# RandomMike1280/AlphaZero-Reversi

Hardware: AMD Instinct MI355X
Metric: self-play board-steps/sec @ 800 sims/move, 8x8 Reversi (higher is better)
Workload: dtype u64 rules + f32 NN (fp32 as 2-part f16 split on MFMA)

## Files before the change

### alphazero-reversi_amd/csrc/rvz_engine_host.h

```cpp
#pragma once
#include <hip/hip_runtime.h>
#include <stdint.h>

#include <string>
#include <utility>
#include <vector>

#include "../../include/rvz.h"
#include "rvz_host.hip.h"
#include "rvz_search.hip.h"

using namespace rvz;

struct rvz_engine {
    rvz_config cfg;
    int BS, NSQ, NPOL, E, M;
    hipStream_t stream = nullptr;
    int next_batch = 0;
    int32_t* live_buf = nullptr;
    unsigned long long* live_total = nullptr;
    int live_dirty = 0;
    int searching = 0;
    int pending = 0;
    const float* pend_policy = nullptr;
    const float* pend_value = nullptr;
    int pend_is_logits = 0;
    int64_t counters[2] = {0, 0};
    View v;
    unsigned long long* stats_buf = nullptr;
    int timing = 0;
    std::vector<hipEvent_t> ev_pool;
    size_t ev_used = 0;
    std::vector<std::pair<int, size_t>> ev_marks;
    std::vector<void*> allocs;
    std::string err;
    unsigned long long* tab = nullptr;
    unsigned* tclaim = nullptr;
    unsigned* tgen = nullptr;
    int64_t tslots = 0;
    int tmaxd = 0;
    const void* tab_blob = nullptr;
    double gate_frac = -1.0, gate_us = 0.0, gate_late_us = 0.0;
    int32_t* noise_err = nullptr;
    void* open_buf = nullptr;
};

#define RVZ_HIP(call, e)                                                                   \
    do {                                                                                   \
        hipError_t _s = (call);                                                            \
        if (_s != hipSuccess) {                                                            \
            (e)->err = std::string(#call) + ": " + hipGetErrorString(_s);                  \
            return RVZ_EHIP;                                                               \
        }                                                                                  \
    } while (0)

static int launch_check(rvz_engine* e, const char* what) {
    hipError_t s = hipGetLastError();
    if (s != hipSuccess) {
        e->err = std::string(what) + ": " + hipGetErrorString(s);
        return RVZ_EHIP;
    }
    e->counters[1] += 1;
    return RVZ_OK;
}

static int grid_games(int G) { return (G + WPB - 1) / WPB; }

template <class... P, class... A>
static void launch_games_unchecked(rvz_engine* e, void (*k8)(P...), void (*k6)(P...), A... args) {
    launch_bs_unchecked(e->BS, k8, k6, dim3(grid_games(e->v.G)), dim3(WPB * WAVE), e->stream,
                        args...);
}
template <class... P, class... A>
static int launch_games(rvz_engine* e, const char* what, void (*k8)(P...), void (*k6)(P...),
                        A... args) {
// ... 27 lines not shown
```

### alphazero-reversi_amd/csrc/rvz_play.hip

```cpp
#include <hip/hip_runtime.h>
#include <math.h>
#include <stdint.h>
#include <stdio.h>
#include <stdlib.h>

#include <string>
#include <vector>

#include "../../include/rvz.h"
#include "rvz_engine_host.h"
#include "rvz_h2.hip.h"
#include "rvz_host.hip.h"
#include "rvz_play.hip.h"
#include "rvz_search.hip.h"
#include "rvz_trace.h"

using namespace rvz;


__global__ void k_table_bump(unsigned* gen) {
    if (threadIdx.x == 0) atomicAdd(gen, 1u);
}

int table_bump(rvz_engine* e) {
    if (!e->tgen) return RVZ_OK;
    hipLaunchKernelGGL(k_table_bump, dim3(1), dim3(64), 0, e->stream, e->tgen);
    RVZ_HIP(hipGetLastError(), e);
    return RVZ_OK;
}

void table_free(rvz_engine* e) {
    for (void* p : {(void*)e->tab, (void*)e->tclaim, (void*)e->tgen})
        if (p) (void)hipFree(p);
    e->tab = nullptr;
    e->tclaim = nullptr;
    e->tgen = nullptr;
    e->tslots = 0;
    e->tab_blob = nullptr;
}

extern "C" {

int rvz_play_gate(rvz_engine* e, double fraction, double timeout_us, double late_us) {
    if (!e || !(fraction <= 1.0) || !(timeout_us >= 0.0) || !(late_us >= 0.0) ||
        timeout_us > 1e6 || late_us > 1e6) {
        if (e) e->err = "rvz_play_gate: fraction <= 1 (< 0: the default), 0 <= us <= 1e6";
        return RVZ_EINVAL;
    }
    e->gate_frac = fraction;
    e->gate_us = timeout_us;
    e->gate_late_us = late_us;
    return RVZ_OK;
}

int rvz_play_table(rvz_engine* e, int64_t slots, int32_t max_discs) {
    if (!e) return RVZ_EINVAL;
    if (slots != 0 && (slots < 1024 || (slots & (slots - 1)) != 0 || slots > (1ll << 30) ||
                       max_discs < 4)) {
        e->err = "rvz_play_table: slots a power of two in [1024, 2^30] (or 0), max_discs >= 4";
        return RVZ_EINVAL;
    }
    RVZ_HIP(hipStreamSynchronize(e->stream), e);
    if (slots == e->tslots && slots != 0) {
        e->tmaxd = max_discs;
        return table_bump(e);
    }
    table_free(e);
    if (slots == 0) return RVZ_OK;
    const size_t stride = e->BS == 8 ? TabGeo<8>::STRIDE : TabGeo<6>::STRIDE;
    if (hipMalloc(reinterpret_cast<void**>(&e->tab), (size_t)slots * stride * 8) != hipSuccess ||
        hipMalloc(reinterpret_cast<void**>(&e->tclaim), (size_t)slots * 4) != hipSuccess ||
        hipMalloc(reinterpret_cast<void**>(&e->tgen), 4) != hipSuccess) {
        table_free(e);
        e->err = "hipMalloc failed (rvz_play_table)";
        return RVZ_ENOMEM;
    }
    hipError_t st = hipMemset(e->tab, 0, (size_t)slots * stride * 8);
    if (st == hipSuccess) st = hipMemset(e->tclaim, 0, (size_t)slots * 4);
    if (st == hipSuccess) st = hipMemsetD32(e->tgen, 1u, 1);
    if (st == hipSuccess) st = hipDeviceSynchronize();
    if (st != hipSuccess) {
        table_free(e);
        e->err = std::string("rvz_play_table init: ") + hipGetErrorString(st);
        return RVZ_EHIP;
    }
    e->tslots = slots;
    e->tmaxd = max_discs;
    return RVZ_OK;
}

#ifdef RVZ_WALK_STATS
int rvz_play_walk_read(int32_t n_games, uint64_t* out) {
    const int n = n_games < WALK_STATS_MAX ? n_games : WALK_STATS_MAX;
    std::vector<unsigned long long> a, b;
    if (take_rows(g_wtime, n, a) != RVZ_OK || take_rows(g_ftime, n, b) != RVZ_OK) return RVZ_EHIP;
    for (int i = 0; i < n; ++i) {
        for (int k = 0; k < 5; ++k) out[(size_t)i * 9 + k] = a[(size_t)i * 5 + k];
        for (int k = 0; k < 4; ++k) out[(size_t)i * 9 + 5 + k] = b[(size_t)i * 4 + k];
    }
    return RVZ_OK;
}
#endif

struct PlayScratch {
    int64_t q_next, q_done, gate, queue, x, need, work, logits, value, total;
};
static PlayScratch play_scratch(int64_t G, int NSQ, int NPOL) {
    const auto al4 = [](int64_t n) { return (n + 3) / 4 * 4; };
    int64_t at = 0;
    const auto take = [&](int64_t words) { const int64_t o = at; at += al4(words); return o; };
    PlayScratch s;
    s.q_next = take(4);
    s.q_done = take(2 * al4(G));
    s.gate = take(8 * 32);
    s.queue = at;
    s.x = take(G * 3 * NSQ);
    s.need = take(G);
    s.work = take(G * 192);
    s.logits = take(G * NPOL);
    s.value = take(G);
    s.total = at;
    return s;
}
int64_t rvz_play_scratch_size(const rvz_engine* e) {
    if (!e) return RVZ_EINVAL;
    return play_scratch(e->v.G, e->NSQ, e->NPOL).total;
}

#ifndef RVZ_PLAY_GROUP
#define RVZ_PLAY_GROUP 4
#endif
#ifndef RVZ_PLAY_GATE_FRAC
#define RVZ_PLAY_GATE_FRAC 0.8
#endif
#ifndef RVZ_PLAY_GATE_US
#define RVZ_PLAY_GATE_US 400.0
#endif
#ifndef RVZ_PLAY_GATE_LATE_US
#define RVZ_PLAY_GATE_LATE_US 200.0
#endif
extern "C++" {
template <class T>
static int play_launch(rvz_engine* e, const View& v, const PlayArgs& pa) {
    constexpr int F = T::F, BS = T::BS;
    int cus = 0;
    if (hipDeviceGetAttribute(&cus, hipDeviceAttributeMultiprocessorCount, e->cfg.device) !=
            hipSuccess || cus <= 0)
        cus = 256;
    PlayArgs a = pa;
    const int slots = cus * T::OCC;
    dim3 grid;
    if (a.q_next) {
        if (a.gpw <= 0) a.gpw = RVZ_PLAY_GROUP;
        if (a.gpw > play_gpw_max<F, BS>()) a.gpw = play_gpw_max<F, BS>();
        a.n_groups = (v.G + a.gpw - 1) / a.gpw;
        grid = dim3(a.n_groups < slots ? a.n_groups : slots);
        RVZ_HIP(fill32_async(a.q_next, 0u, (size_t)play_scratch(v.G, e->NSQ, e->NPOL).queue,
                             e->stream), e);
    } else {
        if (a.gpw <= 0) a.gpw = (v.G + slots - 1) / slots;
        if (a.gpw > play_gpw_max<F, BS>()) a.gpw = play_gpw_max<F, BS>();
        a.n_groups = (v.G + a.gpw - 1) / a.gpw;
        grid = dim3(a.n_groups);
    }
    PlayCtx ctx;
    ctx.v = v;
    ctx.a = a;
    hipLaunchKernelGGL((k_play<T::F, T::NB, T::CTW, T::PTW, T::BS, T::OCC>), grid, dim3(256), 0,
                       e->stream, ctx);
    return launch_check(e, "k_play");
}
}

#ifdef RVZ_PLAY_TIMING
int rvz_play_timing_read(uint64_t* host, int n) {
    if (hipMemcpyFromSymbol(host, HIP_SYMBOL(g_play_t), (size_t)n * PLAY_T_SLOTS * 8) != hipSuccess)
        return RVZ_EHIP;
    if (hipMemcpyFromSymbol(host + (size_t)n * PLAY_T_SLOTS, HIP_SYMBOL(g_pass_t),
                            (size_t)n * 6 * 8) != hipSuccess)
        return RVZ_EHIP;
    std::vector<unsigned long long> z((size_t)16384 * PLAY_T_SLOTS, 0ull);
    if (hipMemcpyToSymbol(HIP_SYMBOL(g_pass_t), z.data(), (size_t)16384 * 6 * 8) != hipSuccess)
// ... 67 lines not shown
    pa.need = reinterpret_cast<int32_t*>(a->scratch + sc.need);
    pa.work = a->scratch + sc.work;
    pa.logits = a->scratch + sc.logits;
    pa.value = a->scratch + sc.value;
    pa.n_groups = 0;
    pa.gpw = queue ? -a->games_per_workgroup : a->games_per_workgroup;
    const PlayGate gate = play_gate_setting(e, queue);
    pa.gate_frac = gate.frac;
    pa.gate_t = gate.t;
    pa.gate_late = gate.late;
    pa.spin_limit = 1u << 26;
    if (const char* sl = getenv("RVZ_PLAY_SPIN_LIMIT")) pa.spin_limit = (unsigned)strtoul(sl, nullptr, 10);
    pa.single_pass = 1;
    if (const char* sp = getenv("RVZ_PLAY_SINGLE_PASS")) pa.single_pass = atoi(sp) != 0;
    pa.S = e->cfg.num_simulations;
    pa.B = e->cfg.batch_size;
    pa.skip_last = a->skip_last_eval && pa.S > pa.B ? 1 : 0;
    pa.skip_forced = a->skip_forced_roots && pa.skip_last ? 1 : 0;
    pa.plies = a->plies;
    pa.budget = a->ply_budget;
    pa.temperature = a->temperature;
    pa.reset = a->reset ? 1 : 0;
    pa.seeds = a->seeds;
    pa.stride = a->seed_stride;
    pa.ply_ctr = a->plies_done;
    pa.done = a->games_done;
    pa.out_idx = a->out_idx;
    pa.out_p = a->out_p;
    pa.hist = a->hist;
    pa.rows = reinterpret_cast<unsigned long long*>(a->rows_evaluated);
    pa.unread = reinterpret_cast<unsigned long long*>(a->rows_unread);
    pa.roots_unread = reinterpret_cast<unsigned long long*>(a->roots_unread);
    pa.tstats = reinterpret_cast<unsigned long long*>(a->table_stats);
    pa.rec_black = a->rec_black;
    pa.rec_white = a->rec_white;
    pa.rec_side = a->rec_side;
    pa.rec_p = a->rec_p;
    pa.tab = nullptr;
    pa.tclaim = nullptr;
    pa.tgen = nullptr;
    pa.tmask = 0;
    pa.tmaxd = 0;
    if (e->tab) {
        if (e->tab_blob != a->blob) {
            if (e->tab_blob) {
                hipStreamCaptureStatus cs = hipStreamCaptureStatusNone;
                if (hipStreamIsCapturing(e->stream, &cs) == hipSuccess &&
                    cs != hipStreamCaptureStatusNone) {
                    e->err = "rvz_play: another weight blob than the table's while the stream is "
                             "capturing (play once eagerly with this evaluator before capturing)";
                    return RVZ_EINVAL;
                }
                const int r = table_bump(e);
                if (r != RVZ_OK) return r;
            }
            e->tab_blob = a->blob;
        }
        pa.tab = e->tab;
        pa.tclaim = e->tclaim;
        pa.tgen = e->tgen;
        pa.tmask = (unsigned)(e->tslots - 1);
        pa.tmaxd = e->tmaxd;
    }
    e->searching = 0;
    int r = RVZ_EINVAL;
    h2_tile(e->BS, a->filters, [&](auto t) { r = play_launch<decltype(t)>(e, v, pa); });
// ... 5 lines not shown
```

### alphazero-reversi_amd/csrc/rvz_play.hip.h

```cpp
#pragma once
#include <hip/hip_runtime.h>
#include <stdint.h>

#include "rvz_h2.hip.h"
#include "rvz_resnet_common.hip.h"
#include "rvz_search.hip.h"

namespace rvz {
namespace {

struct PlayArgs {
    const float* prm;
    Layout L;
    const uint16_t* blob;
    int n_blocks;
    float* x;
    int32_t* need;
    float* work;
    float* logits;
    float* value;
    float* ovf;
    int gpw, plies, skip_last, reset, S, B;
    double temperature;
    int64_t* seeds;
    int64_t stride;
    int64_t* ply_ctr;
    int64_t* done;
    int32_t* out_idx;
    double* out_p;
    int32_t* hist;
    unsigned long long* rows;
    const int32_t* budget;
    unsigned spin_limit;
    int single_pass;
    unsigned long long* tab;
    unsigned* tclaim;
    const unsigned* tgen;
    unsigned tmask;
    int tmaxd;
    unsigned long long* tstats;
    unsigned long long* unread;
    uint64_t* rec_black;
    uint64_t* rec_white;
    int32_t* rec_side;
    double* rec_p;
    unsigned* q_next;
    unsigned long long* q_done;
    int n_groups;
    unsigned long long* gate;
    unsigned gate_frac;
    unsigned gate_t;
    unsigned gate_late;
    int skip_forced;
    unsigned long long* roots_unread;
};
constexpr int PLAY_GPW_MAX = 64;
template <int F, int BS>
__host__ __device__ constexpr bool play_heads_lds() { return F == 64 && BS == 8; }
template <int F, int BS>
__host__ __device__ constexpr int play_gpw_max() {
    return play_heads_lds<F, BS>() ? 8 : PLAY_GPW_MAX;
}
enum : int { PF_QUEUED = 1, PF_READY = 2, PF_DONE = 4, PF_EVAL = 8, PF_HELD = 16 };
constexpr int32_t ERR_SCHED = 16;

template <int BS>
struct TabGeo {
    static constexpr int NSQ = Geo<BS>::NSQ;
    static constexpr int NG = NSQ + 8;
    static constexpr int STRIDE = (NG + 7) / 8 * 8;
};
constexpr int TAB_PROBES = 8;

__device__ __forceinline__ uint64_t tab_mix(uint64_t z) {
    z ^= z >> 30;
    z *= 0xbf58476d1ce4e5b9ull;
    z ^= z >> 27;
    z *= 0x94d049bb133111ebull;
    return z ^ (z >> 31);
}
__device__ __forceinline__ uint64_t tab_hash(uint64_t P, uint64_t O, uint64_t V) {
    return tab_mix(P ^ tab_mix(O ^ tab_mix(V + 0x9e3779b97f4a7c15ull)));
}
template <int NSQ>
__device__ __forceinline__ uint32_t tab_key_word(int idx, uint64_t P, uint64_t O, uint64_t V) {
    const int k = idx - (NSQ + 2);
    const uint64_t w = k < 2 ? P : (k < 4 ? O : V);
    return (k & 1) ? (uint32_t)(w >> 32) : (uint32_t)w;
}

template <int BS>
__device__ __forceinline__ int tab_read(const unsigned long long* __restrict__ tab, uint32_t sl,
                                         uint32_t gen, uint64_t P, uint64_t O, uint64_t V,
                                         int lane, uint64_t& x0, uint64_t& x1) {
    using T = TabGeo<BS>;
    constexpr int NSQ = T::NSQ, NG = T::NG;
// ... 111 lines not shown
                           __HIP_MEMORY_SCOPE_AGENT);
}
__device__ __forceinline__ void play_gate(unsigned long long* gate, unsigned frac, unsigned t,
                                          unsigned late) {
    unsigned long long* w = gate_line(gate);
    if (late) {
        const unsigned long long t_open =
            __hip_atomic_load(w + 1, __ATOMIC_RELAXED, __HIP_MEMORY_SCOPE_AGENT);
        if (t_open && __builtin_amdgcn_s_memrealtime() - t_open < late) return;
    }
    const unsigned long long running =
        __hip_atomic_load(w + 2, __ATOMIC_RELAXED, __HIP_MEMORY_SCOPE_AGENT);
    if (running < 4) return;
    const unsigned k = max(1u, (unsigned)((running * frac) >> 16));
    const unsigned long long old =
        __hip_atomic_fetch_add(w, 1ull, __ATOMIC_RELAXED, __HIP_MEMORY_SCOPE_AGENT);
    const unsigned r = (unsigned)(old >> 32);
    if ((unsigned)old + 1u >= k) {
        gate_open(w, r);
        return;
    }
    const unsigned long long t0 = __builtin_amdgcn_s_memrealtime();
    for (;;) {
        __builtin_amdgcn_s_sleep(2);
        const unsigned long long v = __hip_atomic_load(w, __ATOMIC_RELAXED, __HIP_MEMORY_SCOPE_AGENT);
        if ((unsigned)(v >> 32) != r) return;
        if (__builtin_amdgcn_s_memrealtime() - t0 > t) {
            gate_open(w, r);
            return;
        }
    }
}

struct PlayCtx {
    View v;
    PlayArgs a;
};
__device__ __forceinline__ int opaque_tid() {
    int t = threadIdx.x;
    asm volatile("" : "+v"(t));
    return t;
}
__device__ __forceinline__ const PlayCtx& play_ctx() {
    const __attribute__((address_space(4))) char* p =
        (const __attribute__((address_space(4))) char*)__builtin_amdgcn_kernarg_segment_ptr();
    asm volatile("" : "+s"(p));
    return *(const PlayCtx*)p;
}

#ifdef RVZ_PLAY_TIMING
constexpr int PLAY_T_SLOTS = 14;
__device__ unsigned long long g_play_t[16384][PLAY_T_SLOTS];
#define PT_NOW(t) const unsigned long long t = __builtin_amdgcn_s_memtime()
#define PT_ADD(i, v) if (tid == 0 && blockIdx.x < 16384) g_play_t[blockIdx.x][i] += (v)
#else
#define PT_NOW(t)
#define PT_ADD(i, v)
#endif

template <int F, int NBOARD, int CTW, int PTW, int BS, int OCC>
__global__ __launch_bounds__(256) __attribute__((amdgpu_waves_per_eu(OCC, OCC)))
void k_play(PlayCtx ctx0) {
    (void)ctx0;
    using WT = WaveTilesH<F, CTW, PTW>;
    constexpr bool ILV = RVZ_H2_ILV && NBOARD == 2 && BS == 8 && PTW == 4 && WT::CG == 2;
    using GH = GeoH<NBOARD, BS, 64 * CTW * H2_TM / F, ILV>;
    using C = CfgH<F, GH::NPIX>;
    constexpr int NPOL = Geo<BS>::NPOL;
    constexpr bool HLDS = play_heads_lds<F, BS>();
    constexpr int GMAX = play_gpw_max<F, BS>();
    constexpr bool PLAY_SINGLE = F == 64 && NBOARD == 2 && BS == 8 && (PTW & 1) == 0 && HLDS;
    constexpr int HROW = heads_in_floats(BS) / 16;
    constexpr int SP_BYTES = WPB * (NPOL + 7) * 8;
    static_assert(heads_in_floats(BS) * 4 <= C::RMAX, "heads rows fit");
    static_assert(SP_BYTES + WPB * 624 * 4 <= C::RMAX, "act / reset scratch fits");
    __shared__ __attribute__((aligned(16))) char smem[C::BYTES];
    __shared__ int st_k[GMAX];
    __shared__ int st_f[GMAX];
    __shared__ int st_p[GMAX];
    __shared__ uint64_t st_bits[GMAX * 3];
    __shared__ uint64_t q_bits[(GMAX + NBOARD) * 3];
    __shared__ __attribute__((aligned(16))) float hin[HLDS ? GMAX * HROW : 4];
    __shared__ int q_rows[GMAX + 16];
    __shared__ int s_nq;
    __shared__ float vpart[4][16];
    __shared__ int s_task[2];
    __shared__ unsigned s_tgen;
    const int tid = threadIdx.x;
    const int wave = __builtin_amdgcn_readfirstlane(tid >> 6);
    int E, G, gpw, queue, task_plies;
    {
        const PlayCtx& c = play_ctx();
        E = c.v.E;
        G = c.v.G;
        gpw = c.a.gpw;
        queue = c.a.q_next != nullptr;
        task_plies = queue ? 1 : c.a.plies;
    }
    bool ovf = false;
    __shared__ unsigned s_cnt[5];
    if (tid < 5) s_cnt[tid] = 0u;
    if (tid == 0) {
        const PlayArgs& a = play_ctx().a;
        s_tgen = a.tab ? __hip_atomic_load(a.tgen, __ATOMIC_RELAXED, __HIP_MEMORY_SCOPE_AGENT) : 0u;
    }
    double* sp = reinterpret_cast<double*>(smem) + wave * (NPOL + 7);
    uint32_t* key = reinterpret_cast<uint32_t*>(smem + SP_BYTES) + wave * 624;
    if constexpr (F >= 128 && BS == 8) {
        const PlayArgs& a = play_ctx().a;
        if (tid == 0 && a.gate_frac > 0) gate_running(a.gate, 1);
    }
    PT_NOW(t_start);
    for (int task_i = 0;; ++task_i) {
        int gi, ply0;
        if (!queue) {
            if (task_i > 0) break;
            gi = blockIdx.x;
            ply0 = 0;
        } else {
            PT_NOW(t_q0);
            if (wave == 0) {
                const PlayCtx& c = play_ctx();
                const PlayArgs& a = c.a;
                const int n = a.n_groups;
                const unsigned plies = (unsigned)a.plies;
                const int rot = (int)((unsigned long long)blockIdx.x * (unsigned)n / gridDim.x);
                int tg = -1, tp = 0;
                bool stop = __hip_atomic_load(c.v.err, __ATOMIC_RELAXED,
                                              __HIP_MEMORY_SCOPE_AGENT) & ERR_SCHED;
                unsigned spins = 0;
                while (!stop) {
                    unsigned long long best = ~0ull;
                    bool left = false;
                    for (int i = tid; i < n; i += 64) {
// ... 96 lines not shown
                            root_meta = v.meta[(size_t)g * v.M];
                            root_n = v.nodes[(size_t)g * v.M].n;
                        } else if (v.memo) {
                            carry = v.carry[g];
                        }
                        if (f & PF_READY) {
                            WT_NOW(ft_e);
                            const ExpIn x = expand_load<BS>(v, g, lane, a.logits, a.value);
                            const int rn =
                                expand_backup_phase<BS>(v, g, lane, x, 1, &root_meta, ab);
                            if (rn >= 0) root_n = rn;
                            f &= ~PF_READY;
                            FT_ADD(0, ft_e);
                        }
                        const int bsz = min(a.B, a.S - k * a.B);
                        const bool unread = a.skip_last && !first && m_nchild(root_meta) >= E - 1;
                        const Forced fz{first && a.skip_forced ? E : 0, a.S, a.B};
                        const int copies = select_phase<BS, float>(v, g, lane, first, bsz, k, root,
                                                                   root_meta, root_n, carry, a.x,
                                                                   a.need, ab, st_bits + 3 * j,
                                                                   unread, fz);
                        if (copies <= -2) {
                            k = E;
                            const int left = -2 - copies;
                            if (lane == 0) {
                                if (left & 255) atomicAdd(&s_cnt[3], (unsigned)(left & 255));
                                if (left >> 8) atomicAdd(&s_cnt[4], 1u);
                            }
                            continue;
                        }
                        ++k;
                        if (copies < 0 && k < E && lane == 0) atomicAdd(&s_cnt[3], 1u);
                        if (copies > 0 && !(k == E && a.skip_last)) {
                            if (a.tab) {
                                const uint64_t P = st_bits[3 * j], O = st_bits[3 * j + 1],
                                               Vb = st_bits[3 * j + 2];
                                WT_NOW(ft_t);
                                const bool hit = __popcll(P | O) <= a.tmaxd &&
                                                 tab_lookup<BS>(a, s_tgen, P, O, Vb, lane, g);
                                WT_ADD(0, ft_t);
                                if (hit) {
                                    __builtin_amdgcn_fence(__ATOMIC_SEQ_CST, "workgroup");
                                    f |= PF_READY;
                                    if (lane == 0) atomicAdd(&s_cnt[1], 1u);
                                    continue;
                                }
                            }
                            f |= PF_QUEUED;
                            break;
                        }
                        continue;
                    }
                    WT_NOW(ft_a);
                    bool over = false;
                    double* outp = a.out_p;
                    if (a.rec_black) {
                        const size_t ri = (size_t)(ply0 + np) * v.G + g;
                        if (lane == 0) {
                            a.rec_black[ri] = v.black[g];
                            a.rec_white[ri] = v.white[g];
                            a.rec_side[ri] = v.status[(size_t)g * 4];
                        }
                        outp = a.rec_p + (size_t)(ply0 + np) * v.G * Geo<BS>::NPOL;
                    }
                    const int idx = act_game<BS>(v, g, lane, sp, (f & PF_READY) ? 1 : 2,
                                                 a.logits, 1, a.value, a.temperature, nullptr, 1,
                                                 a.out_idx, outp, &over);
                    f &= ~PF_READY;
                    int64_t sd = 0;
                    if (lane == 0) {
                        if (idx >= 0) a.ply_ctr[g] += 1;
                        if (a.hist) a.hist[(size_t)(ply0 + np) * v.G + g] = idx;
                        if (a.reset && over) {
                            a.done[g] += 1;
                            sd = a.seeds[g] + a.stride;
                            a.seeds[g] = sd;
                        }
                    }
                    if (a.reset && over) {
                        sd = __shfl(sd, 0);
                        reset_game<BS>(v, g, lane, (uint32_t)(sd & 0xFFFFFFFFll), key);
                    }
                    FT_ADD(1, ft_a);
                    ++np;
                    k = 0;
                    if (np >= task_plies || (a.budget && ply0 + np >= a.budget[g])) {
                        f |= PF_DONE;
                        break;
                    }
                }
                FT_ADD(2, ft_step);
                if (lane == 0) {
                    st_k[j] = k;
                    st_f[j] = f;
                    st_p[j] = np;
                }
            }
            __syncthreads();
            PT_NOW(t_c1);
            PT_ADD(0, t_c1 - t_c0);
            PT_ADD(4, 1);
            if (tid == 0) {
                int n = 0;
                for (int j = 0; j < ng; ++j)
                    if (st_f[j] & PF_QUEUED) ++n;
                int hold = n > NBOARD ? n % NBOARD : 0;
                for (int j = ng - 1; j >= 0; --j) {
                    const int fj = st_f[j];
                    if (!(fj & PF_QUEUED)) continue;
                    if (hold > 0 && !(fj & PF_HELD)) {
                        st_f[j] = fj | PF_HELD;
                        --hold;
                    } else {
                        st_f[j] = (fj & ~PF_HELD) | PF_EVAL;
                    }
                }
                n = 0;
                for (int j = 0; j < ng; ++j)
                    if (st_f[j] & PF_EVAL) {
                        for (int ch = 0; ch < 3; ++ch) q_bits[3 * n + ch] = st_bits[3 * j + ch];
                        q_rows[n++] = g0 + j;
                    }
                for (int i = n; i < n + 16; ++i) q_rows[i] = -1;
                for (int i = 3 * n; i < 3 * (n + NBOARD); ++i) q_bits[i] = 0;
                s_nq = n;
            }
            __syncthreads();
            const int nq = __builtin_amdgcn_readfirstlane(s_nq);
            if (nq == 0) break;
            if (tid == 0) s_cnt[0] += (unsigned)nq;
            PT_NOW(t_c2);

            for (int p0 = 0; p0 < nq; p0 += NBOARD) {
                if constexpr (F >= 128 && BS == 8) {
                    if (play_ctx().a.gate_frac > 0) {
                        if (tid == 0) {
                            const PlayArgs& a = play_ctx().a;
                            play_gate(a.gate, a.gate_frac, a.gate_t, a.gate_late);
                        }
                        __syncthreads();
                    }
                }
                const PlayArgs& a = play_ctx().a;
                PT_NOW(t_p0);
                bool single = false;
                if constexpr (PLAY_SINGLE)
                    single = a.single_pass &&
                             __builtin_amdgcn_readfirstlane(q_rows[p0 + 1]) < 0;
                if (single) {
                    if constexpr (PLAY_SINGLE) {
                        const int t = opaque_tid();
                        ovf |= h2_pass_single<F, CTW, PTW / 2, BS>(
                                   smem, q_bits + 3 * p0, a.prm, a.blob, a.n_blocks, hin, p0, nq,
                                   t, t & 63, __builtin_amdgcn_readfirstlane(t >> 6)) != 0;
                    }
                } else {
                    int gb[NBOARD];
// ... 85 lines not shown
    if (queue && tid == 0) {
        const PlayCtx& c = play_ctx();
        const PlayArgs& a = c.a;
        unsigned spins = 0;
        bool stop = __hip_atomic_load(c.v.err, __ATOMIC_RELAXED, __HIP_MEMORY_SCOPE_AGENT) &
                    ERR_SCHED;
        while (!stop && (int)__hip_atomic_load(a.q_next, __ATOMIC_RELAXED,
                                               __HIP_MEMORY_SCOPE_AGENT) < a.n_groups) {
            __builtin_amdgcn_s_sleep(4);
            ++spins;
            if (spins > a.spin_limit ||
                ((spins & 1023u) == 0 &&
                 (__hip_atomic_load(c.v.err, __ATOMIC_RELAXED, __HIP_MEMORY_SCOPE_AGENT) &
                  ERR_SCHED))) {
                atomicOr(c.v.err, ERR_SCHED);
                stop = true;
            }
        }
    }
    float* ovw = play_ctx().a.ovf;
    if (ovf && ovw) *ovw = 1.0f;
    unsigned long long* rows = play_ctx().a.rows;
    __syncthreads();
    if (rows && tid == 0) atomicAdd(rows, (unsigned long long)s_cnt[0]);
    unsigned long long* ts = play_ctx().a.tstats;
    if (ts && tid == 0) {
        if (s_cnt[1]) atomicAdd(ts, (unsigned long long)s_cnt[1]);
        if (s_cnt[2]) atomicAdd(ts + 1, (unsigned long long)s_cnt[2]);
    }
    unsigned long long* un = play_ctx().a.unread;
    if (un && tid == 0 && s_cnt[3]) atomicAdd(un, (unsigned long long)s_cnt[3]);
    unsigned long long* ur = play_ctx().a.roots_unread;
    if (ur && tid == 0 && s_cnt[4]) atomicAdd(ur, (unsigned long long)s_cnt[4]);
}

}
}
```

### alphazero-reversi_amd/csrc/rvz_search.hip.h

```cpp
#pragma once
#include <hip/hip_runtime.h>
#include <math.h>
#include <stdint.h>

#include "../../include/rvz.h"
#include "rvz_dirichlet.hip.h"
#include "rvz_openings.hip.h"
#include "rvz_philox.hip.h"
#include "rvz_pow.hip.h"
#include "rvz_rules.hip.h"
#include "rvz_wave_dpp.hip.h"

namespace rvz {
namespace {

constexpr int WAVE = 64;
constexpr int WPB = 4;
constexpr int PATH_CAP = 64;
constexpr int RNG_DRAWS = 64;

}

struct Node {
    int32_t n;
// ... 557 lines not shown
            if (leaf_bits) {
                if (lane == 0) {
                    leaf_bits[0] = mine(sim);
                    leaf_bits[1] = theirs(sim);
                    leaf_bits[2] = V;
                }
            } else if (lane < NSQ) {
                XT* row = leaf_x + (size_t)r * 3 * NSQ;
                const uint64_t P = mine(sim), O = theirs(sim);
                row[lane] = (XT)(float)((P >> lane) & 1ull);
                row[NSQ + lane] = (XT)(float)((O >> lane) & 1ull);
                row[2 * NSQ + lane] = (XT)(float)((V >> lane) & 1ull);
            }
            if (lane < plen) v.path[g * PATH_CAP + lane] = path_reg;
            if (lane == 0) {
                v.leaf_legal[g] = V;
                v.leaf_meta[g] = m;
            }
            WT_ADD(4, tl0);
            ab += 3ull * NSQ * sizeof(XT) + 4ull * plen + 12;
            break;
        }
    }
    if (lane == 0) {
        need[g] = copies;
        v.pend[g] = copies;
        v.plen[g] = plen;
    }
    ab += 12;
    return copies;
}

template <int BS>
__device__ __forceinline__ int root_visits(const View& v, int g, int lane) {
    constexpr int NSQ = Geo<BS>::NSQ;
    const Node* nodes = v.nodes + (size_t)g * v.M;
    const uint32_t m0 = v.meta[(size_t)g * v.M];
    const uint64_t V = v.root_legal[g];
    const int nch = m_nchild(m0);
    if (nch == 0 || lane >= NSQ) return 0;
    if (!((V >> lane) & 1ull)) return 0;
    const int idx = __popcll(V & ((1ull << lane) - 1ull));
    return nodes[1 + m_block(m0) * NSQ + idx].n;
}

__device__ __forceinline__ double np_power(double x, double e) {
    if (e == 1.0) return x;
    if (e == 2.0) return x * x;
    if (e == 0.5) return sqrt(x);
    if (e == -1.0) return 1.0 / x;
    if (e == 0.0) return 1.0;
    return rvz_pow::pow_cr(x, e);
}

template <int BS, class Draw>
__device__ __forceinline__ int select_action(int n, int npass, int lane, double* s,
                                             double temperature, Draw&& draw, double& p,
                                             double& ppass, int& drew) {
    constexpr int NSQ = Geo<BS>::NSQ, NPOL = Geo<BS>::NPOL;
    constexpr int NMAIN = NPOL - NPOL % 8;
    const int total = wave_sum_i(lane < NSQ ? n : 0) + npass;
    p = (lane < NSQ && total > 0) ? (double)n / (double)total : 0.0;
    ppass = npass != 0 ? (double)npass / (double)total : 0.0;
    if (temperature > 0.0 && (__any(p != 0.0) || ppass != 0.0)) {
        const double ex = 1.0 / temperature;
        const double t = lane < NSQ ? np_power(p, ex) : 0.0;
// ... 165 lines not shown
```

### alphazero-reversi_amd/rvz/_lib.py

```python
from __future__ import annotations

import ctypes as C
import math
import numbers
import os

import torch

_HERE = os.path.dirname(os.path.abspath(__file__))
LIB_PATH = os.environ.get("RVZ_LIB", os.path.join(_HERE, "librvz.so"))

RVZ_OK, RVZ_DONE = 0, 1
RVZ_LEAF_F32, RVZ_LEAF_BF16 = 0, 1
RVZ_DRAWS = 64
RVZ_SOLVE_MAX_EMPTIES = 14
RVZ_SOLVE_NOT_A_MOVE, RVZ_SOLVE_ABANDONED = -128, -127
RVZ_AB_MAX_DEPTH = 12
RVZ_AB_WIN = 20000
RVZ_AB_HEUR_MAX = 16000


class RvzError(RuntimeError):
    pass

# ... 78 lines not shown
                                            C.c_uint64, C.c_uint64, _P, _P, _P, _P, _P, _P, _P]),
    "rvz_replay_is_weight_scratch_size": (C.c_int64, [C.c_int32]),
    "rvz_replay_is_weight": (C.c_int, [C.c_int32, _P, _P, C.c_double, _P, _P, _P, _P]),
    "rvz_replay_priority_scratch_size": (C.c_int64, [C.c_int32]),
    "rvz_replay_priority": (C.c_int, [C.c_int32, _P, C.c_int32, _P, _P, C.c_double, C.c_double,
                                      C.c_int32, C.c_double, C.c_double, C.c_double, _P, _P, _P,
                                      _P, _P]),
    "rvz_replay_stale_scratch_size": (C.c_int64, [C.c_int32, C.c_int32]),
    "rvz_replay_stale": (C.c_int, [C.c_int32, _P, C.c_int32, C.c_int32, C.c_int32, C.c_int32,
                                   C.c_int32, _P, C.c_int64, _P, _P, _P]),
    "rvz_replay_roots": (C.c_int, [C.c_int32, C.c_int32, _P, _P, C.c_int32, _P, _P, _P, _P, _P,
                                   _P]),
    "rvz_replay_refresh_scratch_size": (C.c_int64, [C.c_int32]),
    "rvz_replay_refresh": (C.c_int, [C.c_int32, C.c_int32, _P, _P, C.c_int32, _P, _P, _P,
                                     C.c_int32, _P, C.c_int64, _P, _P]),
    "rvz_records_scratch_size": (C.c_int64, [C.c_int32, C.c_int32]),
    "rvz_records_games": (C.c_int, [C.c_int32, C.c_int32, C.c_int32, _P, _P, _P, _P, _P, C.c_int32,
                                    _P, _P, _P, _P, _P, _P, _P, _P, _P, _P]),
    "rvz_records_final": (C.c_int, [C.c_int32, C.c_int32, C.c_int32, _P, _P, _P, _P, C.c_int32,
                                    _P, _P, _P, _P, _P, _P, _P]),
    "rvz_openings_scratch_size": (C.c_int64, [C.c_int32, C.c_int32]),
    "rvz_openings": (C.c_int, [C.c_int32, C.c_int32, C.c_int32, _P, _P, _P, _P, _P, _P, _P]),
    "rvz_env_openings": (C.c_int, [_P, C.c_int32, _P, _P, _P, C.c_uint32]),
    "rvz_opening_index": (C.c_int, [C.c_int32, C.c_int32, _P, C.c_uint32, _P, _P]),
    "rvz_loss_scratch_size": (C.c_int64, [C.c_int32, C.c_int32]),
    "rvz_policy_value_loss": (C.c_int, [C.c_int32, C.c_int32, _P, _P, _P, _P, _P, C.c_double,
                                        C.c_double, _P, _P, _P, _P, _P, _P]),
    "rvz_ownership_loss_scratch_size": (C.c_int64, [C.c_int32, C.c_int32]),
    "rvz_ownership_loss": (C.c_int, [C.c_int32, C.c_int32, _P, _P, _P, _P, _P, _P, _P, _P]),
    "rvz_play_scratch_size": (C.c_int64, [_P]),
    "rvz_play": (C.c_int, [_P, _P]),
    "rvz_play_table": (C.c_int, [_P, C.c_int64, C.c_int32]),
    "rvz_play_gate": (C.c_int, [_P, C.c_double, C.c_double, C.c_double]),
    "rvz_counters": (C.c_int, [_P, C.POINTER(C.c_int64)]),
    "rvz_stats_enable": (C.c_int, [_P, C.c_int32]),
    "rvz_stats_read": (C.c_int, [_P, C.POINTER(C.c_int64)]),
    "rvz_timing_enable": (C.c_int, [_P, C.c_int32]),
    "rvz_timing_read": (C.c_int, [_P, C.POINTER(C.c_double), C.POINTER(C.c_int32)]),
    "rvz_tree_nodes": (C.c_int, [_P]),
    "rvz_tree_export": (C.c_int, [_P, _P, _P]),
    "rvz_footprint": (C.c_int, [_P, C.POINTER(C.c_int64), C.POINTER(C.c_int64)]),
    "rvz_resnet_params_size": (C.c_int64, [C.c_int32, C.c_int32, C.c_int32]),
    "rvz_resnet_work_size": (C.c_int64, [C.c_int32]),
    "rvz_resnet_heads_fc": (C.c_int, [C.c_int32, _P, C.c_int32, _P, C.c_int32, C.c_int32, _P, _P,
                                      _P]),
    "rvz_resnet_h2_size": (C.c_int64, [C.c_int32, C.c_int32]),
    "rvz_resnet_h2_weights": (C.c_int, [_P, C.c_int32, C.c_int32, _P, _P]),
    "rvz_resnet_trunk_h2": (C.c_int, [C.c_int32, _P, C.c_int32, _P, _P, C.c_int32, C.c_int32,
                                      _P, _P]),
    "rvz_resnet_fwd_h2": (C.c_int, [C.c_int32, _P, C.c_int32, _P, _P, C.c_int32, C.c_int32, _P,
                                    _P, _P, _P]),
}

_lib = None


class PlayArgs(C.Structure):
    _fields_ = [("params", C.c_void_p), ("blob", C.c_void_p), ("filters", C.c_int32),
                ("blocks", C.c_int32), ("scratch", C.c_void_p), ("ovf", C.c_void_p),
                ("plies", C.c_int32), ("skip_last_eval", C.c_int32), ("reset", C.c_int32),
                ("games_per_workgroup", C.c_int32), ("temperature", C.c_double),
                ("seeds", C.c_void_p), ("seed_stride", C.c_int64), ("plies_done", C.c_void_p),
                ("games_done", C.c_void_p), ("out_idx", C.c_void_p), ("out_p", C.c_void_p),
                ("hist", C.c_void_p), ("rows_evaluated", C.c_void_p),
                ("ply_budget", C.c_void_p), ("table_stats", C.c_void_p),
                ("rec_black", C.c_void_p), ("rec_white", C.c_void_p), ("rec_side", C.c_void_p),
# ... 123 lines not shown
```

### alphazero-reversi_amd/rvz/engine.py

```python
from __future__ import annotations

import ctypes as C
from typing import Callable, Optional, Sequence, Tuple

import torch

from . import _lib
from ._lib import (RVZ_DONE, RVZ_LEAF_BF16, RVZ_LEAF_F32, RvzError, check, check_board_size,
                   ptr)

U64 = 0xFFFFFFFFFFFFFFFF
SOLVE_MAX_EMPTIES = _lib.RVZ_SOLVE_MAX_EMPTIES
SOLVE_NOT_A_MOVE = _lib.RVZ_SOLVE_NOT_A_MOVE
SOLVE_ABANDONED = _lib.RVZ_SOLVE_ABANDONED
AB_MAX_DEPTH = _lib.RVZ_AB_MAX_DEPTH
AB_WIN = _lib.RVZ_AB_WIN
AB_HEUR_MAX = _lib.RVZ_AB_HEUR_MAX


def to_signed64(x: int) -> int:
    x &= U64
    return x - (1 << 64) if x >> 63 else x


# ... 193 lines not shown
    def solve_moves_wld(self, max_empties: int = SOLVE_MAX_EMPTIES, node_limit: int = 2 ** 24,
                        order_min_empties: Optional[int] = None):
        b, w, st = self._env_snapshot()
        if order_min_empties is None:
            order_min_empties = WLD_ORDER_MIN_EMPTIES
        return solve_moves_wld(b, w, st, self.board_size, max_empties, node_limit,
                               order_min_empties)

    def alphabeta(self, depth: int = 4, weights: Optional[Sequence[int]] = None,
                  node_limit: int = 2 ** 24):
        b, w, st = self._env_snapshot()
        return alphabeta(b, w, st, self.board_size, depth, weights, node_limit)

    def legal(self) -> torch.Tensor:
        self._stream()
        out = torch.empty(self.n_games, dtype=torch.int64, device=self.device)
        self._call("rvz_env_legal", ptr(out))
        return out

    def apply(self, sq: torch.Tensor) -> torch.Tensor:
        self._stream()
        s = sq.to(self.device, torch.int32).contiguous()
        ok = torch.empty(self.n_games, dtype=torch.int32, device=self.device)
        self._call("rvz_env_apply", ptr(s), ptr(ok))
        return ok

    def play_buffers(self, evaluator=None):
        if getattr(self, "play_rows", None) is None:
            self.play_rows = torch.zeros(1, dtype=torch.int64, device=self.device)
            self.table_stats = torch.zeros(2, dtype=torch.int64, device=self.device)
            self.play_unread = torch.zeros(1, dtype=torch.int64, device=self.device)
        if getattr(self, "play_roots_unread", None) is None:
            self.play_roots_unread = torch.zeros(1, dtype=torch.int64, device=self.device)
        n = self.lib.rvz_play_scratch_size(self._h)
        sc = getattr(self, "_play_scratch", None)
        if sc is None or sc.numel() < n:
            self._play_scratch = torch.zeros(n, dtype=torch.float32, device=self.device)
        if evaluator is not None and hasattr(evaluator, "ovf_word"):
            evaluator.ovf_word()

    def play(self, evaluator, plies: int, temperature: float, seeds: torch.Tensor, stride: int,
             plies_done: torch.Tensor, games_done: torch.Tensor, reset: bool = True,
             skip_last_eval: bool = False, hist: Optional[torch.Tensor] = None,
             games_per_workgroup: int = 0, budget: Optional[torch.Tensor] = None,
             records=None, skip_forced_roots: bool = False):
        from .network import LeafEvaluator
        if not isinstance(evaluator, LeafEvaluator):
            raise RvzError("play() runs the h2 LeafEvaluator inside the launch; another "
                           "evaluator goes through search() / act()")
        if evaluator.board_size != self.board_size or evaluator.device != self.device:
            raise RvzError("play(): the evaluator's board size / device differ from the engine's")
        for t, dt in ((seeds, torch.int64), (plies_done, torch.int64), (games_done, torch.int64)):
            if t.dtype != dt or t.numel() != self.n_games or not t.is_contiguous():
                raise RvzError("play: seeds / plies_done / games_done int64 [n_games]")
        if hist is not None and (hist.dtype != torch.int32 or hist.shape != (plies, self.n_games)
                                 or not hist.is_contiguous()):
            raise RvzError("play: hist int32 [plies, n_games]")
        if budget is not None and (budget.dtype != torch.int32 or budget.numel() != self.n_games
                                   or not budget.is_contiguous()
                                   or budget.device != self.device):
            raise RvzError("play: budget int32 [n_games] on the engine's device")
        rec = (None,) * 4
        if records is not None and hist is None:
            raise RvzError("play: records need hist (the moves of the recorded plies)")
        if records is not None:
            rb, rw, rs, rp = records
            G = self.n_games
            if not (rb.dtype == rw.dtype == torch.int64 and rs.dtype == torch.int32
                    and rp.dtype == torch.float64 and rb.shape == rw.shape == rs.shape
                    == (plies, G) and rp.shape == (plies, G, self.npol)
                    and all(t.is_contiguous() and t.device == self.device
                            for t in (rb, rw, rs, rp))):
                raise RvzError("play: records = (black int64, white int64 [plies, G], side int32 "
                               "[plies, G], p float64 [plies, G, npol]) on the engine's device")
            rec = tuple(t.data_ptr() for t in records)
        n = self.lib.rvz_play_scratch_size(self._h)
        ready = (getattr(self, "play_rows", None) is not None and
                 getattr(self, "play_roots_unread", None) is not None and
                 getattr(self, "_play_scratch", None) is not None and
                 self._play_scratch.numel() >= n and getattr(evaluator, "_ovf", None) is not None)
        if not ready:
            if torch.cuda.is_current_stream_capturing():
                raise RvzError("play() inside a graph capture before its buffers exist: call "
                               "Engine.play_buffers(evaluator) (or one eager play) first")
            self.play_buffers(evaluator)
        sc = self._play_scratch
        self._bind(evaluator)
        a = _lib.PlayArgs(evaluator.params.data_ptr(), evaluator.wsplit.data_ptr(),
                          evaluator.filters, evaluator.n_blocks, sc.data_ptr(),
                          evaluator.ovf_word().data_ptr(), int(plies), int(bool(skip_last_eval)),
                          int(bool(reset)), int(games_per_workgroup), float(temperature),
                          seeds.data_ptr(), int(stride), plies_done.data_ptr(),
                          games_done.data_ptr(), self.idx_buf.data_ptr(), self.p_buf.data_ptr(),
                          hist.data_ptr() if hist is not None else None,
                          self.play_rows.data_ptr(),
                          budget.data_ptr() if budget is not None else None,
                          self.table_stats.data_ptr(), *rec, self.play_unread.data_ptr(),
                          int(bool(skip_forced_roots)), self.play_roots_unread.data_ptr())
        self._stream()
        self._call("rvz_play", C.byref(a))

    def _bind(self, evaluator):
        evs = self.__dict__.setdefault("_evaluators", [])
        if not any(e is evaluator for e in evs):
            evs.append(evaluator)
            reg = getattr(evaluator, "bind_engine", None)
            if reg is not None:
                reg(self)

    def table(self, slots: int = 1 << 20, max_discs: int = 14):
        self._stream()
        self._call("rvz_play_table", int(slots), int(max_discs))
        self.table_slots = int(slots)

    def play_gate(self, fraction: float = -1.0, timeout_us: float = 0.0, late_us: float = 0.0):
        self._call("rvz_play_gate", float(fraction), float(timeout_us), float(late_us))

    def root_noise(self, alpha: float, epsilon: float, salt: int = 0):
        _lib.check_noise_args(alpha, epsilon)
        self._call("rvz_search_root_noise", float(alpha), float(epsilon), int(salt) & 0xFFFFFFFF)
        self.noise = (float(alpha), float(epsilon), int(salt) & 0xFFFFFFFF)

    def openings(self, black: Optional[torch.Tensor], white: Optional[torch.Tensor] = None,
                 side: Optional[torch.Tensor] = None, salt: int = 0):
        self._stream()
        if black is None:
            self._call("rvz_env_openings", 0, None, None, None, 0)
            self.pool = None
            return
        if white is None or side is None:
            raise RvzError("openings: black, white and side, or None for off")
        n = black.numel()
        if n < 1 or black.dim() != 1 or white.shape != (n,) or side.shape != (n,) or \
# ... 299 lines not shown
```

### include/rvz.h

```cpp
#ifndef RVZ_H
#define RVZ_H
#include <stdint.h>

#ifdef __cplusplus
extern "C" {
#endif

#define RVZ_OK 0
#define RVZ_DONE 1
#define RVZ_EINVAL (-22)
#define RVZ_ENOMEM (-12)
#define RVZ_EHIP (-5)
#define RVZ_EDEVICE (-71)

#define RVZ_LEAF_F32 0
#define RVZ_LEAF_BF16 1

#define RVZ_LIVE_STRIPE 128
#define RVZ_LIVE_PITCH 16

typedef struct rvz_engine rvz_engine;

typedef struct rvz_config {
    int32_t board_size;
// ... 224 lines not shown
    const float *params;
    const uint16_t *blob;
    int32_t filters;
    int32_t blocks;
    float *scratch;
    float *ovf;
    int32_t plies;
    int32_t skip_last_eval;
    int32_t reset;
    int32_t games_per_workgroup;
    double temperature;
    int64_t *seeds;
    int64_t seed_stride;
    int64_t *plies_done;
    int64_t *games_done;
    int32_t *out_idx;
    double *out_p;
    int32_t *hist;
    int64_t *rows_evaluated;
    const int32_t *ply_budget;
    int64_t *table_stats;
    uint64_t *rec_black;
    uint64_t *rec_white;
    int32_t *rec_side;
    double *rec_p;
    int64_t *rows_unread;
    int32_t skip_forced_roots;
    int64_t *roots_unread;
} rvz_play_args;
int64_t rvz_play_scratch_size(const rvz_engine *e);
int rvz_play(rvz_engine *e, const rvz_play_args *a);
int rvz_play_table(rvz_engine *e, int64_t slots, int32_t max_discs);
int rvz_play_gate(rvz_engine *e, double fraction, double timeout_us, double late_us);

typedef struct rvz_timer rvz_timer;
int rvz_timer_create(int32_t n_events, rvz_timer **out);
int rvz_timer_record(rvz_timer *t, int32_t i, void *hip_stream);
int rvz_timer_elapsed(rvz_timer *t, int32_t i, int32_t j, float *ms );
void rvz_timer_destroy(rvz_timer *t);

int rvz_counters(const rvz_engine *e, int64_t *out2 );
int rvz_stats_enable(rvz_engine *e, int32_t on);
int rvz_stats_read(rvz_engine *e, int64_t *out3 );
int rvz_timing_enable(rvz_engine *e, int32_t on);
int rvz_timing_read(rvz_engine *e, double *out_ms , int32_t *out_n );
int rvz_tree_nodes(const rvz_engine *e);
int rvz_tree_export(rvz_engine *e, void *nodes_out, uint32_t *meta_out);
int rvz_footprint(const rvz_engine *e, int64_t *bytes_tree, int64_t *bytes_env);

int64_t rvz_resnet_params_size(int32_t board, int32_t filters, int32_t blocks);
int64_t rvz_resnet_work_size(int32_t n);
int rvz_resnet_heads_fc(int32_t board, const float *work, int32_t n, const float *params,
                        int32_t filters, int32_t blocks, float *logits, float *value,
                        void *hip_stream);

int64_t rvz_resnet_h2_size(int32_t filters, int32_t blocks);
int rvz_resnet_h2_weights(const float *params, int32_t filters, int32_t blocks, uint16_t *blob,
                          void *hip_stream);
int rvz_resnet_fwd_h2(int32_t board, const float *x, int32_t n, const float *params,
                      const uint16_t *blob, int32_t filters, int32_t blocks, float *work,
                      float *logits, float *value, void *hip_stream);
int rvz_resnet_trunk_h2(int32_t board, const float *x, int32_t n, const float *params,
                        const uint16_t *blob, int32_t filters, int32_t blocks, float *work,
                        void *hip_stream);
int32_t rvz_resnet_h2_grid(int32_t board, int32_t filters, int32_t n);
int rvz_resnet_fwd_h2_ex(int32_t board, const float *x, int32_t n, const float *params,
// ... 15 lines not shown
```

Baseline: 1.839 million.

## Fill odd NN batch slot with speculative look-ahead child evaluation

When the play kernel's eval queue holds an odd number of boards (the NN evaluates boards in pairs), it now picks a queued game, finds its next fresh root child with legal moves, and evaluates that position in the otherwise empty slot. The result and a key are stashed in scratch, and the next time that game needs an eval whose board matches the key, the cached logits/value are copied instead of queuing a new eval. This targets the wasted half-batch and the extra eval round-trips. The cost is extra wave work to simulate the candidate child and key-checking overhead, and the pre-evaluation is wasted when the prediction misses. Mode 2 also drops the hold logic, and the feature is on by default and selectable through an env var and an API.

```diff
diff --git a/alphazero-reversi_amd/csrc/rvz_engine_host.h b/alphazero-reversi_amd/csrc/rvz_engine_host.h
--- a/alphazero-reversi_amd/csrc/rvz_engine_host.h
+++ b/alphazero-reversi_amd/csrc/rvz_engine_host.h
@@ -41,6 +41,8 @@
     int tmaxd = 0;
     const void* tab_blob = nullptr;
     double gate_frac = -1.0, gate_us = 0.0, gate_late_us = 0.0;
+    int ahead = -1;
+    int64_t* ahead_stats = nullptr;
     int32_t* noise_err = nullptr;
     void* open_buf = nullptr;
 };
diff --git a/alphazero-reversi_amd/csrc/rvz_play.hip b/alphazero-reversi_amd/csrc/rvz_play.hip
--- a/alphazero-reversi_amd/csrc/rvz_play.hip
+++ b/alphazero-reversi_amd/csrc/rvz_play.hip
@@ -50,6 +50,21 @@
     e->gate_frac = fraction;
     e->gate_us = timeout_us;
     e->gate_late_us = late_us;
+    return RVZ_OK;
+}
+
+int rvz_play_ahead(rvz_engine* e, int32_t mode) {
+    if (!e || mode > 2) {
+        if (e) e->err = "rvz_play_ahead: mode 0, 1 or 2 (< 0: the default)";
+        return RVZ_EINVAL;
+    }
+    e->ahead = mode;
+    return RVZ_OK;
+}
+
+int rvz_play_ahead_stats(rvz_engine* e, int64_t* stats) {
+    if (!e) return RVZ_EINVAL;
+    e->ahead_stats = stats;
     return RVZ_OK;
 }
 
@@ -104,6 +119,7 @@
 
 struct PlayScratch {
     int64_t q_next, q_done, gate, queue, x, need, work, logits, value, total;
+    int64_t ah_logits, ah_value, ah_key;
 };
 static PlayScratch play_scratch(int64_t G, int NSQ, int NPOL) {
     const auto al4 = [](int64_t n) { return (n + 3) / 4 * 4; };
@@ -120,6 +136,9 @@
     s.logits = take(G * NPOL);
     s.value = take(G);
     s.total = at;
+    s.ah_logits = s.x;
+    s.ah_value = s.x + al4(2 * G * NPOL);
+    s.ah_key = s.work;
     return s;
 }
 int64_t rvz_play_scratch_size(const rvz_engine* e) {
@@ -129,6 +148,9 @@
 
 #ifndef RVZ_PLAY_GROUP
 #define RVZ_PLAY_GROUP 4
+#endif
+#ifndef RVZ_PLAY_AHEAD_DEFAULT
+#define RVZ_PLAY_AHEAD_DEFAULT 1
 #endif
 #ifndef RVZ_PLAY_GATE_FRAC
 #define RVZ_PLAY_GATE_FRAC 0.8
@@ -148,6 +170,18 @@
             hipSuccess || cus <= 0)
         cus = 256;
     PlayArgs a = pa;
+    if constexpr (play_ahead_shape<F, T::NB, BS>()) {
+        static_assert(3 * Geo<BS>::NSQ >= 2 * Geo<BS>::NPOL + 8, "ahead rows fit");
+        if (a.ahead) {
+            const PlayScratch sc = play_scratch(v.G, e->NSQ, e->NPOL);
+            float* scratch = a.x - sc.x;
+            a.logits = scratch + sc.ah_logits;
+            a.value = scratch + sc.ah_value;
+            a.ah_key = reinterpret_cast<uint64_t*>(scratch + sc.ah_key);
+        }
+    } else {
+        a.ahead = 0;
+    }
     const int slots = cus * T::OCC;
     dim3 grid;
     if (a.q_next) {
@@ -281,6 +315,11 @@
     pa.unread = reinterpret_cast<unsigned long long*>(a->rows_unread);
     pa.roots_unread = reinterpret_cast<unsigned long long*>(a->roots_unread);
     pa.tstats = reinterpret_cast<unsigned long long*>(a->table_stats);
+    pa.ahead = e->ahead < 0 ? RVZ_PLAY_AHEAD_DEFAULT : e->ahead;
+    if (const char* ah = getenv("RVZ_PLAY_AHEAD")) pa.ahead = atoi(ah);
+    if (pa.ahead < 0 || pa.ahead > 2 || !pa.single_pass) pa.ahead = 0;
+    pa.ah_key = nullptr;
+    pa.ah_stats = reinterpret_cast<unsigned long long*>(e->ahead_stats);
     pa.rec_black = a->rec_black;
     pa.rec_white = a->rec_white;
     pa.rec_side = a->rec_side;
diff --git a/alphazero-reversi_amd/csrc/rvz_play.hip.h b/alphazero-reversi_amd/csrc/rvz_play.hip.h
--- a/alphazero-reversi_amd/csrc/rvz_play.hip.h
+++ b/alphazero-reversi_amd/csrc/rvz_play.hip.h
@@ -53,6 +53,9 @@
     unsigned gate_late;
     int skip_forced;
     unsigned long long* roots_unread;
+    int ahead;
+    uint64_t* ah_key;
+    unsigned long long* ah_stats;
 };
 constexpr int PLAY_GPW_MAX = 64;
 template <int F, int BS>
@@ -61,7 +64,11 @@
 __host__ __device__ constexpr int play_gpw_max() {
     return play_heads_lds<F, BS>() ? 8 : PLAY_GPW_MAX;
 }
-enum : int { PF_QUEUED = 1, PF_READY = 2, PF_DONE = 4, PF_EVAL = 8, PF_HELD = 16 };
+template <int F, int NBOARD, int BS>
+__host__ __device__ constexpr bool play_ahead_shape() {
+    return NBOARD == 2 && play_heads_lds<F, BS>();
+}
+enum : int { PF_QUEUED = 1, PF_READY = 2, PF_DONE = 4, PF_EVAL = 8, PF_HELD = 16, PF_AHEAD = 32 };
 constexpr int32_t ERR_SCHED = 16;
 
 template <int BS>
@@ -239,6 +246,22 @@
     }
 }
 
+template <int BS>
+__device__ __forceinline__ bool ahead_take(const PlayArgs& a, int G, int g, const uint64_t* bits,
+                                           int lane) {
+    constexpr int NSQ = Geo<BS>::NSQ, NPOL = Geo<BS>::NPOL;
+    const bool ne = lane < 3 && a.ah_key[3 * (size_t)g + lane] != bits[lane];
+    if (__ballot(ne) != 0ull) return false;
+    const float* src = a.logits + (size_t)(G + g) * NPOL;
+    float* row = a.logits + (size_t)g * NPOL;
+    if (lane < NSQ) row[lane] = src[lane];
+    if (lane == 0) {
+        row[NSQ] = src[NSQ];
+        a.value[g] = a.value[G + g];
+    }
+    return true;
+}
+
 struct PlayCtx {
     View v;
     PlayArgs a;
@@ -256,11 +279,13 @@
 }
 
 #ifdef RVZ_PLAY_TIMING
-constexpr int PLAY_T_SLOTS = 14;
+constexpr bool PLAY_TIMED = true;
+constexpr int PLAY_T_SLOTS = 16;
 __device__ unsigned long long g_play_t[16384][PLAY_T_SLOTS];
 #define PT_NOW(t) const unsigned long long t = __builtin_amdgcn_s_memtime()
 #define PT_ADD(i, v) if (tid == 0 && blockIdx.x < 16384) g_play_t[blockIdx.x][i] += (v)
 #else
+constexpr bool PLAY_TIMED = false;
 #define PT_NOW(t)
 #define PT_ADD(i, v)
 #endif
@@ -277,6 +302,7 @@
     constexpr bool HLDS = play_heads_lds<F, BS>();
     constexpr int GMAX = play_gpw_max<F, BS>();
     constexpr bool PLAY_SINGLE = F == 64 && NBOARD == 2 && BS == 8 && (PTW & 1) == 0 && HLDS;
+    constexpr bool PLAY_AHEAD = PLAY_SINGLE && play_ahead_shape<F, NBOARD, BS>();
     constexpr int HROW = heads_in_floats(BS) / 16;
     constexpr int SP_BYTES = WPB * (NPOL + 7) * 8;
     static_assert(heads_in_floats(BS) * 4 <= C::RMAX, "heads rows fit");
@@ -305,8 +331,9 @@
         task_plies = queue ? 1 : c.a.plies;
     }
     bool ovf = false;
-    __shared__ unsigned s_cnt[5];
-    if (tid < 5) s_cnt[tid] = 0u;
+    constexpr int NCNT = PLAY_AHEAD ? 7 : 5;
+    __shared__ unsigned s_cnt[NCNT];
+    if (tid < NCNT) s_cnt[tid] = 0u;
     if (tid == 0) {
         const PlayArgs& a = play_ctx().a;
         s_tgen = a.tab ? __hip_atomic_load(a.tgen, __ATOMIC_RELAXED, __HIP_MEMORY_SCOPE_AGENT) : 0u;
@@ -469,6 +496,15 @@
                         ++k;
                         if (copies < 0 && k < E && lane == 0) atomicAdd(&s_cnt[3], 1u);
                         if (copies > 0 && !(k == E && a.skip_last)) {
+                            if constexpr (PLAY_AHEAD) {
+                                if ((f & PF_AHEAD) &&
+                                    ahead_take<BS>(a, G, g, st_bits + 3 * j, lane)) {
+                                    __builtin_amdgcn_fence(__ATOMIC_SEQ_CST, "workgroup");
+                                    f = (f & ~PF_AHEAD) | PF_READY;
+                                    if (lane == 0) atomicAdd(&s_cnt[6], 1u);
+                                    continue;
+                                }
+                            }
                             if (a.tab) {
                                 const uint64_t P = st_bits[3 * j], O = st_bits[3 * j + 1],
                                                Vb = st_bits[3 * j + 2];
@@ -504,6 +540,7 @@
                                                  a.logits, 1, a.value, a.temperature, nullptr, 1,
                                                  a.out_idx, outp, &over);
                     f &= ~PF_READY;
+                    if constexpr (PLAY_AHEAD) f &= ~PF_AHEAD;
                     int64_t sd = 0;
                     if (lane == 0) {
                         if (idx >= 0) a.ply_ctr[g] += 1;
@@ -537,11 +574,37 @@
             PT_NOW(t_c1);
             PT_ADD(0, t_c1 - t_c0);
             PT_ADD(4, 1);
+            bool ah_found = false;
+            int ah_j = 0;
+            uint64_t ah_P = 0, ah_O = 0, ah_V = 0;
+            if constexpr (PLAY_AHEAD) {
+                const PlayCtx& c = play_ctx();
+                if (wave == 0 && (c.a.ahead != 0 || PLAY_TIMED)) {
+                    const int lane = opaque_tid() & 63;
+                    const int fj = lane < ng ? st_f[lane] : 0;
+                    const int n = __popcll(__ballot((fj & PF_QUEUED) != 0));
+                    const bool holds = n > NBOARD && __ballot((fj & PF_QUEUED) && !(fj & PF_HELD));
+                    if ((n & 1) && (!holds || c.a.ahead == 2 || PLAY_TIMED)) {
+                        uint64_t cand = __ballot((fj & PF_QUEUED) && !(fj & PF_AHEAD));
+                        while (cand != 0ull && !ah_found) {
+                            ah_j = 63 - __clzll((long long)cand);
+                            cand &= ~(1ull << ah_j);
+                            ah_found = ahead_child<BS>(c.v, g0 + ah_j, st_k[ah_j], E, lane, ah_P,
+                                                       ah_O, ah_V);
+                        }
+                    }
+                }
+            }
             if (tid == 0) {
                 int n = 0;
                 for (int j = 0; j < ng; ++j)
                     if (st_f[j] & PF_QUEUED) ++n;
                 int hold = n > NBOARD ? n % NBOARD : 0;
+                if constexpr (PLAY_AHEAD) {
+                    PT_ADD(14, n & 1);
+                    PT_ADD(15, (n & 1) && ah_found);
+                    if (ah_found && play_ctx().a.ahead == 2) hold = 0;
+                }
                 for (int j = ng - 1; j >= 0; --j) {
                     const int fj = st_f[j];
                     if (!(fj & PF_QUEUED)) continue;
@@ -560,6 +623,21 @@
                     }
                 for (int i = n; i < n + 16; ++i) q_rows[i] = -1;
                 for (int i = 3 * n; i < 3 * (n + NBOARD); ++i) q_bits[i] = 0;
+                if constexpr (PLAY_AHEAD) {
+                    const PlayArgs& a = play_ctx().a;
+                    if (ah_found && a.ahead != 0 && (n & 1)) {
+                        const int g = g0 + ah_j;
+                        q_bits[3 * n] = ah_P;
+                        q_bits[3 * n + 1] = ah_O;
+                        q_bits[3 * n + 2] = ah_V;
+                        q_rows[n++] = G + g;
+                        a.ah_key[3 * (size_t)g] = ah_P;
+                        a.ah_key[3 * (size_t)g + 1] = ah_O;
+                        a.ah_key[3 * (size_t)g + 2] = ah_V;
+                        st_f[ah_j] |= PF_AHEAD;
+                        s_cnt[5] += 1u;
+                    }
+                }
                 s_nq = n;
             }
             __syncthreads();
@@ -711,7 +789,14 @@
     if (un && tid == 0 && s_cnt[3]) atomicAdd(un, (unsigned long long)s_cnt[3]);
     unsigned long long* ur = play_ctx().a.roots_unread;
     if (ur && tid == 0 && s_cnt[4]) atomicAdd(ur, (unsigned long long)s_cnt[4]);
-}
-
-}
-}
+    if constexpr (PLAY_AHEAD) {
+        unsigned long long* as = play_ctx().a.ah_stats;
+        if (as && tid == 0 && s_cnt[5]) {
+            atomicAdd(as, (unsigned long long)s_cnt[5]);
+            atomicAdd(as + 1, (unsigned long long)s_cnt[6]);
+        }
+    }
+}
+
+}
+}
diff --git a/alphazero-reversi_amd/csrc/rvz_search.hip.h b/alphazero-reversi_amd/csrc/rvz_search.hip.h
--- a/alphazero-reversi_amd/csrc/rvz_search.hip.h
+++ b/alphazero-reversi_amd/csrc/rvz_search.hip.h
@@ -613,6 +613,41 @@
 }
 
 template <int BS>
+__device__ __forceinline__ bool ahead_child(const View& v, int g, int k, int E, int lane,
+                                            uint64_t& P, uint64_t& O, uint64_t& V) {
+    constexpr int NSQ = Geo<BS>::NSQ;
+    const Node* nodes = v.nodes + (size_t)g * v.M;
+    const uint32_t* meta = v.meta + (size_t)g * v.M;
+    const uint32_t m0 = meta[0];
+    const int nch = m_nchild(m0);
+    if (m_term(m0) || nch == 0 || nch >= E - 1 || k < 1 || k > nch) return false;
+    const int base = 1 + m_block(m0) * NSQ;
+    Node c;
+    uint32_t cm = 0;
+    c.n = 1; c.c = 0.0f;
+    if (lane < nch) {
+        c = nodes[base + lane];
+        cm = meta[base + lane];
+    }
+    const bool fresh = lane < nch && lane >= k - 1 && c.n == 0 &&
+                       !(v.memo && link_ok(__float_as_uint(c.c)));
+    const GameS root = load_game(v, g);
+    if (root.over) return false;
+    for (uint64_t rest = __ballot(fresh); rest != 0ull; rest &= rest - 1ull) {
+        const int ci = __ffsll((unsigned long long)rest) - 1;
+        GameS sim = root;
+        make_move_wave<BS>(sim, m_sq((uint32_t)lane_bcast((int)cm, ci)), lane);
+        V = legal_wave<BS>(mine(sim), theirs(sim), lane);
+        if (V != 0ull) {
+            P = mine(sim);
+            O = theirs(sim);
+            return true;
+        }
+    }
+    return false;
+}
+
+template <int BS>
 __device__ __forceinline__ int root_visits(const View& v, int g, int lane) {
     constexpr int NSQ = Geo<BS>::NSQ;
     const Node* nodes = v.nodes + (size_t)g * v.M;
diff --git a/alphazero-reversi_amd/rvz/_lib.py b/alphazero-reversi_amd/rvz/_lib.py
--- a/alphazero-reversi_amd/rvz/_lib.py
+++ b/alphazero-reversi_amd/rvz/_lib.py
@@ -134,6 +134,8 @@
     "rvz_play": (C.c_int, [_P, _P]),
     "rvz_play_table": (C.c_int, [_P, C.c_int64, C.c_int32]),
     "rvz_play_gate": (C.c_int, [_P, C.c_double, C.c_double, C.c_double]),
+    "rvz_play_ahead": (C.c_int, [_P, C.c_int32]),
+    "rvz_play_ahead_stats": (C.c_int, [_P, _P]),
     "rvz_counters": (C.c_int, [_P, C.POINTER(C.c_int64)]),
     "rvz_stats_enable": (C.c_int, [_P, C.c_int32]),
     "rvz_stats_read": (C.c_int, [_P, C.POINTER(C.c_int64)]),
diff --git a/alphazero-reversi_amd/rvz/engine.py b/alphazero-reversi_amd/rvz/engine.py
--- a/alphazero-reversi_amd/rvz/engine.py
+++ b/alphazero-reversi_amd/rvz/engine.py
@@ -249,6 +249,9 @@
             self.play_unread = torch.zeros(1, dtype=torch.int64, device=self.device)
         if getattr(self, "play_roots_unread", None) is None:
             self.play_roots_unread = torch.zeros(1, dtype=torch.int64, device=self.device)
+        if getattr(self, "play_ahead", None) is None:
+            self.play_ahead = torch.zeros(2, dtype=torch.int64, device=self.device)
+            self._call("rvz_play_ahead_stats", self.play_ahead.data_ptr())
         n = self.lib.rvz_play_scratch_size(self._h)
         sc = getattr(self, "_play_scratch", None)
         if sc is None or sc.numel() < n:
@@ -294,6 +297,7 @@
         n = self.lib.rvz_play_scratch_size(self._h)
         ready = (getattr(self, "play_rows", None) is not None and
                  getattr(self, "play_roots_unread", None) is not None and
+                 getattr(self, "play_ahead", None) is not None and
                  getattr(self, "_play_scratch", None) is not None and
                  self._play_scratch.numel() >= n and getattr(evaluator, "_ovf", None) is not None)
         if not ready:
@@ -316,6 +320,9 @@
                           int(bool(skip_forced_roots)), self.play_roots_unread.data_ptr())
         self._stream()
         self._call("rvz_play", C.byref(a))
+
+    def ahead(self, mode: int = -1):
+        self._call("rvz_play_ahead", int(mode))
 
     def _bind(self, evaluator):
         evs = self.__dict__.setdefault("_evaluators", [])
diff --git a/include/rvz.h b/include/rvz.h
--- a/include/rvz.h
+++ b/include/rvz.h
@@ -280,6 +280,8 @@
 int rvz_play(rvz_engine *e, const rvz_play_args *a);
 int rvz_play_table(rvz_engine *e, int64_t slots, int32_t max_discs);
 int rvz_play_gate(rvz_engine *e, double fraction, double timeout_us, double late_us);
+int rvz_play_ahead(rvz_engine *e, int32_t mode);
+int rvz_play_ahead_stats(rvz_engine *e, int64_t *stats);
 
 typedef struct rvz_timer rvz_timer;
 int rvz_timer_create(int32_t n_events, rvz_timer **out);
```

Result: faster. 1.858 million (median of 6 runs) (+1.0%).
